# nguyenduchuyiu/marl-delivery

Measured on AMD Instinct MI355X. Metric: agent-steps/sec (whole node), map1 5-agent 4096 envs, 1/2/4/8 MI355X, higher is better.
Workload: dtype int32+fp64

## Files before the change

marl-delivery_amd/csrc/mdl_device.hpp:

```cpp
#pragma once
#include <hip/hip_runtime.h>
#include <stdint.h>

#if !defined(MDL_PROFILING_BUILD) && \
    (defined(MDL_EXP_NOWAIT) || defined(MDL_EXP_NOTUPLES) || defined(MDL_EXP_NOLDS) || defined(MDL_ABLATE) || \
     defined(MDL_STAMPS))
#error "MDL_EXP_NOWAIT / MDL_EXP_NOTUPLES / MDL_EXP_NOLDS / MDL_ABLATE / MDL_STAMPS need -DMDL_PROFILING_BUILD"
#endif
#ifndef MDL_ABLATE
#define MDL_ABLATE 0
#endif

namespace mdl {

constexpr int WAVE = 64;
constexpr int MT_N = 624;
constexpr int MT_M = 397;
constexpr int MAX_MAPS = 8;
constexpr int PKG_PAD = 256;

enum : int { ST_NONE = 0, ST_WAITING = 1, ST_IN_TRANSIT = 2, ST_DELIVERED = 3 };
enum : int { MV_S = 0, MV_L = 1, MV_R = 2, MV_U = 3, MV_D = 4, MV_OTHER = 5 };
enum : int { SH_PICK = 0, SH_ONTIME, SH_LATE, SH_CLOSER, SH_WPICK, SH_WDROP, SH_STUCK, SH_IDLE, SH_AWAY };

struct MapDesc {
    int H, W, nfree;
    int grid_off;
    int free_off;
    int rank_off;
    float inv_hw;
    int bits_off;
    int mvc_off;
};

struct __align__(16) EnvScalars {
    int32_t t;
    uint32_t ctr;
    double total;
};
enum : uint32_t { RT_MOVE = 1u, RT_ONTIME = 2u, RT_LATE = 4u };

enum : uint32_t { PS_STATUS = 3u, PS_PRESENT = 4u, PS_TRANSIT = 8u, PS_SURVIVOR = 16u, PS_FLAGS = 31u };
constexpr int PS_RANK_SHIFT = 5;

constexpr uint32_t ORD_EPISODE = 0x400u;

struct DevParams {
    int E, A, P, T;
    double move_cost, delivery_reward, delay_reward;
    double cost_sum[9];
    float shaping[9];
    int stale;
    int obsT, MO, MP, MR, MPs;
    int n_maps;
    int key32_dsh;
    MapDesc maps[MAX_MAPS];
    const uint8_t* grids;
    const uint8_t* movevalid;
    const uint8_t* movevalid_cell;
    const uint32_t* gridbits;
    const uint16_t* free_cells;
    const uint16_t* rank;
    const uint8_t* env_map;
    uint32_t* rob;
    uint64_t* pkg;
    uint16_t* pstate;
    EnvScalars* es;
    uint32_t* mt;
    int32_t* mt_pos;
    uint64_t* trk;
    double* ep_total;
    int32_t* ep_len;
    const double* obs_recip;
    int obs_plane_words;
    int obs_small;
    int key7_dsh;
    double cost_fold[65];
};

__host__ __device__ __forceinline__ uint32_t rob_pack(int cell, int carry, uint32_t valid_mask ) {
    return (uint32_t)cell | ((uint32_t)carry << 16) | ((valid_mask & 0x1eu) << 26);
}
__host__ __device__ __forceinline__ int rob_cell(uint32_t w) { return (int)(w & 0xffffu); }
__host__ __device__ __forceinline__ int rob_carry(uint32_t w) { return (int)((w >> 16) & 0x7ffu); }
__host__ __device__ __forceinline__ uint32_t rob_valid(uint32_t w) { return (w >> 26) & 0x1eu; }

__device__ __forceinline__ int lane_id() { return (int)(threadIdx.x & 63); }
__device__ __forceinline__ int wave_id() { return __builtin_amdgcn_readfirstlane((int)(threadIdx.x >> 6)); }

__device__ __forceinline__ int xcd_slot(int b, int nb) { return (b & 7) * (nb >> 3) + min(b & 7, nb & 7) + (b >> 3); }
__device__ __forceinline__ int xcd_block() {
    return xcd_slot((int)blockIdx.x, (int)gridDim.x);
}

__device__ __forceinline__ void wave_sync() {
    __builtin_amdgcn_fence(__ATOMIC_RELEASE, "wavefront");
    __builtin_amdgcn_wave_barrier();
    __builtin_amdgcn_fence(__ATOMIC_ACQUIRE, "wavefront");
}

__device__ __forceinline__ uint64_t ballot(bool p) { return __ballot(p); }

#define GLOBAL __attribute__((address_space(1)))
typedef unsigned int u32x4 __attribute__((ext_vector_type(4)));

template <class T>
__device__ __forceinline__ void pin(T& v) { asm volatile("" : "+s"(v)); }

__device__ __forceinline__ int rdl(int v, int j) { return __builtin_amdgcn_readlane(v, j); }
__device__ __forceinline__ float rdlf(float v, int j) {
    return __int_as_float(__builtin_amdgcn_readlane(__float_as_int(v), j));
}
__device__ __forceinline__ int uni(int v) { return __builtin_amdgcn_readfirstlane(v); }

__device__ __forceinline__ uint32_t lmask(bool b) {
    uint32_t x = b ? ~0u : 0u;
    asm("" : "+v"(x));
    return x;
}
__device__ __forceinline__ uint32_t vbit(uint64_t m, int lane) { return 0u - (uint32_t)((m >> lane) & 1ull); }
__device__ __forceinline__ float fmask(uint32_t m, float a) { return __uint_as_float(m & __float_as_uint(a)); }
__device__ __forceinline__ float fpick(uint32_t m, float a, float b) {
    return __uint_as_float((m & __float_as_uint(a)) | (~m & __float_as_uint(b)));
}
__device__ __forceinline__ int ipick(uint32_t m, int a, int b) { return (int)((m & (uint32_t)a) | (~m & (uint32_t)b)); }

__device__ __forceinline__ int popc64(uint64_t m) { return __popcll(m); }
__device__ __forceinline__ int ffs64(uint64_t m) { return __ffsll((long long)m) - 1; }
__device__ __forceinline__ uint64_t lanemask_lt() {
    int l = lane_id();
    return l == 0 ? 0ull : (~0ull >> (64 - l));
}

__device__ __forceinline__ uint32_t wave_min_u32(uint32_t v) {
    const int id = (int)0xffffffff;
    uint32_t t;
    t = (uint32_t)__builtin_amdgcn_update_dpp(id, (int)v, 0x111, 0xf, 0xf, false); v = t < v ? t : v;
    t = (uint32_t)__builtin_amdgcn_update_dpp(id, (int)v, 0x112, 0xf, 0xf, false); v = t < v ? t : v;
    t = (uint32_t)__builtin_amdgcn_update_dpp(id, (int)v, 0x114, 0xf, 0xf, false); v = t < v ? t : v;
    t = (uint32_t)__builtin_amdgcn_update_dpp(id, (int)v, 0x118, 0xf, 0xf, false); v = t < v ? t : v;
    t = (uint32_t)__builtin_amdgcn_update_dpp(id, (int)v, 0x142, 0xa, 0xf, false); v = t < v ? t : v;
    t = (uint32_t)__builtin_amdgcn_update_dpp(id, (int)v, 0x143, 0xc, 0xf, false); v = t < v ? t : v;
    return (uint32_t)__builtin_amdgcn_readlane((int)v, 63);
}

__device__ __forceinline__ void wave_min_u32x2(uint32_t u, uint32_t v, uint32_t& mu, uint32_t& mv) {
    const int id = (int)0xffffffff;
    uint32_t a, b;
#define MDL_MIN2(ctl, rm)                                                                  \
    a = (uint32_t)__builtin_amdgcn_update_dpp(id, (int)u, ctl, rm, 0xf, false);            \
    b = (uint32_t)__builtin_amdgcn_update_dpp(id, (int)v, ctl, rm, 0xf, false);            \
    u = a < u ? a : u;                                                                     \
    v = b < v ? b : v;
    MDL_MIN2(0x111, 0xf)
    MDL_MIN2(0x112, 0xf)
    MDL_MIN2(0x114, 0xf)
    MDL_MIN2(0x118, 0xf)
    MDL_MIN2(0x142, 0xa)
    MDL_MIN2(0x143, 0xc)
#undef MDL_MIN2
    mu = (uint32_t)__builtin_amdgcn_readlane((int)u, 63);
    mv = (uint32_t)__builtin_amdgcn_readlane((int)v, 63);
}

__device__ __forceinline__ int wave_min8_lane(int a) { return ((a >> 1) << 4) | ((a & 1) << 3); }
__device__ __forceinline__ uint32_t wave_min8_u32(const uint32_t (&k)[8]) {
    uint32_t m[4], n[2];
#pragma unroll
    for (int i = 0; i < 4; i++) {
        const auto r = __builtin_amdgcn_permlane32_swap(k[i], k[i + 4], false, false);
        m[i] = r[0] < r[1] ? r[0] : r[1];
    }
#pragma unroll
    for (int i = 0; i < 2; i++) {
        const auto r = __builtin_amdgcn_permlane16_swap(m[i], m[i + 2], false, false);
        n[i] = r[0] < r[1] ? r[0] : r[1];
    }
    const bool hi = (lane_id() & 8) != 0;
    const uint32_t keep = hi ? n[1] : n[0], send = hi ? n[0] : n[1];
    const int id = (int)0xffffffff;
    uint32_t t = (uint32_t)__builtin_amdgcn_update_dpp(id, (int)send, 0x128, 0xf, 0xf, false);
    uint32_t v = t < keep ? t : keep;
    t = (uint32_t)__builtin_amdgcn_update_dpp(id, (int)v, 0x141, 0xf, 0xf, false);
    v = t < v ? t : v;
    t = (uint32_t)__builtin_amdgcn_update_dpp(id, (int)v, 0x4E, 0xf, 0xf, false);
    v = t < v ? t : v;
    t = (uint32_t)__builtin_amdgcn_update_dpp(id, (int)v, 0xB1, 0xf, 0xf, false);
    return t < v ? t : v;
}

__device__ __forceinline__ float qdiv_r(int a, double y) { return (float)((double)a * y); }

__device__ __forceinline__ float qdiv(int a, int b) { return (float)a / (float)b; }

__device__ __forceinline__ int fdivi(int i, int d, float inv) {
    int q = (int)((float)i * inv);
    int r = i - q * d;
    if (r < 0) q -= 1;
    else if (r >= d) q += 1;
    return q;
}

__device__ __forceinline__ int cell_r(int pc) { return pc & 255; }
__device__ __forceinline__ int cell_c(int pc) { return (pc >> 8) & 255; }
__device__ __forceinline__ int manhattan(int a, int b) {
    return abs(cell_r(a) - cell_r(b)) + abs(cell_c(a) - cell_c(b));
}
__device__ __forceinline__ int manhattan_sad(int a, int b) {
    return (int)__builtin_amdgcn_sad_u8((uint32_t)a, (uint32_t)b, 0u);
}

__device__ __forceinline__ int pk_start(uint64_t v) { return (int)(v & 0xffff); }
__device__ __forceinline__ int pk_target(uint64_t v) { return (int)((v >> 16) & 0xffff); }
__device__ __forceinline__ int pk_st(uint64_t v) { return (int)((v >> 32) & 0xffff); }
__device__ __forceinline__ int pk_dl(uint64_t v) { return (int)(v >> 48); }
__device__ __forceinline__ uint64_t pk_make(int start, int target, int st, int dl) {
    return (uint64_t)(uint32_t)start | ((uint64_t)(uint32_t)target << 16) | ((uint64_t)(uint32_t)st << 32) |
           ((uint64_t)(uint32_t)dl << 48);
}

__device__ __forceinline__ void decode_action(int a, int fmt, int& mv, int& op) {
    if (fmt == 0) {
        const int q = a / 5;
        const int m = a - 5 * q;
        mv = (0x30214 >> (4 * m)) & 0xf;
        op = q >= 3 ? 0 : q;
    } else {
        mv = a & 7;
        op = (a >> 3) & 3;
        if (mv > MV_OTHER) mv = MV_OTHER;
    }
}

__device__ inline void mt_twist(uint32_t* key) {
    const int lane = lane_id();
    for (int base = 0; base < MT_N; base += WAVE) {
        const int i = base + lane;
        uint32_t v = 0;
        if (i < MT_N) {
            const uint32_t y = (key[i] & 0x80000000u) | (key[i + 1 == MT_N ? 0 : i + 1] & 0x7fffffffu);
            const int k = i + MT_M < MT_N ? i + MT_M : i + MT_M - MT_N;
            v = key[k] ^ (y >> 1) ^ ((y & 1u) ? 0x9908b0dfu : 0u);
        }
        wave_sync();
        if (i < MT_N) key[i] = v;
        wave_sync();
    }
}

struct MTState {
    uint32_t* key;
    int pos;
};

__device__ inline uint32_t mt_next32(MTState& s) {
    if (s.pos == MT_N) {
        mt_twist(s.key);
        s.pos = 0;
    }
    uint32_t y = s.key[s.pos];
    s.pos++;
    y ^= (y >> 11);
    y ^= (y << 7) & 0x9d2c5680u;
    y ^= (y << 15) & 0xefc60000u;
    y ^= (y >> 18);
    return (uint32_t)uni((int)y);
}

__device__ inline int randint(MTState& s, int lo, int hi) {
    const uint32_t rng = (uint32_t)(hi - 1 - lo);
    if (rng == 0) return lo;
    uint32_t mask = rng;
    mask |= mask >> 1; mask |= mask >> 2; mask |= mask >> 4; mask |= mask >> 8; mask |= mask >> 16;
    uint32_t v;
    do {
        v = mt_next32(s) & mask;
    } while (v > rng);
    return lo + (int)v;
}

struct ResetOut {
    int robot_cell;
};

__device__ inline int reset_env(MTState& mt, const DevParams& p, const MapDesc& md, uint64_t* pk, uint8_t* pst,
                                uint64_t* scratch, uint16_t* taken) {
    const int lane = lane_id();
    const int A = p.A, P = p.P;
    const uint16_t* fl = p.free_cells + md.free_off;
    const int F = md.nfree;
    int my_cell = 0;
    int ntk = 0;
    for (int i = 0; i < A; i++) {
        const int k = randint(mt, 0, F - i);
        int idx = k;
        for (int q = 0; q < ntk; q++) {
            const int tq = taken[q];
            if (tq <= idx) idx++;
            else break;
        }
        if (lane == 0) {
            int q = ntk;
            while (q > 0 && taken[q - 1] > idx) {
                taken[q] = taken[q - 1];
                q--;
            }
            taken[q] = (uint16_t)idx;
        }
        ntk++;
        wave_sync();
        if (lane == i) my_cell = fl[idx];
    }
    const int N = md.H;
    const int lim = A < 20 ? A : 20;
    for (int i = 0; i < P; i++) {
        const int s_idx = randint(mt, 0, F);
        int t_idx;
        do {
            t_idx = randint(mt, 0, F);
        } while (t_idx == s_idx);
        const int to_dl = 10 + randint(mt, N / 2, 3 * N);
        const int st = (i <= lim) ? 0 : randint(mt, 1, p.T);
        if (lane == 0) scratch[i] = pk_make(s_idx, t_idx, st, st + to_dl);
    }
    wave_sync();
    for (int j = lane; j < P; j += WAVE) {
        const uint64_t v = scratch[j];
        scratch[j] = pk_make(fl[pk_start(v)], fl[pk_target(v)], pk_st(v), pk_dl(v));
    }
    wave_sync();
    for (int j0 = 0; j0 < P; j0 += WAVE) {
        const int j = j0 + lane;
        uint64_t v = 0;
        int sj = 0, rank = 0;
        if (j < P) {
            v = scratch[j];
            sj = pk_st(v);
        }
        for (int i = 0; i < P; i++) {
            const int si = pk_st(scratch[i]);
            rank += (si < sj) || (si == sj && i < j);
        }
        if (j < P) {
            pk[rank] = v;
        }
    }
    wave_sync();
    for (int j = lane; j < P; j += WAVE) pst[j] = pk_st(pk[j]) == 0 ? ST_WAITING : ST_NONE;
    wave_sync();
    return my_cell;
}

struct TrkFresh {
    static constexpr bool kIdIndexed = true;
    const uint64_t* pk;
    const uint8_t* ps;
    int n;
    __device__ int count() const { return n; }
    __device__ bool present(int j) const { const int s = ps[j] & PS_STATUS; return s == ST_WAITING || s == ST_IN_TRANSIT; }
    __device__ bool in_transit(int j) const { return (ps[j] & PS_STATUS) == ST_IN_TRANSIT; }
    __device__ uint64_t data(int j) const { return pk[j]; }
    __device__ int id(int j) const { return j + 1; }
    __device__ uint32_t order(int j) const { return (uint32_t)j; }
    __device__ int slot_of(int id) const { return (id >= 1 && id <= n && present(id - 1)) ? id - 1 : -1; }
};

struct TrkStale {
    static constexpr bool kIdIndexed = true;
    const uint8_t* ps;
    const uint64_t* td;
    const uint32_t* tq;
    int n;
    __device__ int count() const { return n; }
    __device__ bool present(int j) const { return (ps[j] & PS_PRESENT) != 0; }
    __device__ bool in_transit(int j) const { return (ps[j] & PS_TRANSIT) != 0; }
    __device__ uint64_t data(int j) const { return td[j]; }
    __device__ int id(int j) const { return j + 1; }
    __device__ uint32_t order(int j) const { return tq[j]; }
    __device__ int slot_of(int id) const { return (id >= 1 && id <= n && present(id - 1)) ? id - 1 : -1; }
};

struct TrkView {
    static constexpr bool kIdIndexed = false;
    const int32_t* ids;
    const uint8_t* flag;
    const uint64_t* pk;
    int n;
    __device__ int count() const { return n; }
    __device__ bool present(int j) const { return flag[j] & 1; }
    __device__ bool in_transit(int j) const { return (flag[j] & 2) != 0; }
    __device__ uint64_t data(int j) const { return pk[j]; }
    __device__ int id(int j) const { return ids[j]; }
    __device__ uint32_t order(int j) const { return (uint32_t)j; }
    __device__ int slot_of(int id) const {
        for (int j = 0; j < n; j++)
            if (ids[j] == id) return j;
        return -1;
    }
};

template <class Trk>
__device__ inline float shaped_agent(const Trk& trk, const float* C, bool active, int prev_cell, int prev_carry,
                                     int cur_cell, int cur_carry, int mv, int op, int t_prev, int t_cur) {
    float s = 0.0f;
    const int pslot = (active && prev_carry != 0) ? trk.slot_of(prev_carry) : -1;
    if (prev_carry == 0 && cur_carry != 0) {
        s = s + C[SH_PICK];
    } else if (prev_carry != 0 && cur_carry == 0) {
        if (pslot >= 0) {
            const uint64_t d = trk.data(pslot);
            if (cur_cell == pk_target(d)) s = s + ((t_cur <= pk_dl(d)) ? C[SH_ONTIME] : C[SH_LATE]);
        }
    }
    const bool moved = prev_cell != cur_cell;
    const bool need_can = active && op == 1 && prev_carry == 0 && cur_carry == 0;
    const bool need_near = active && moved && !(prev_carry != 0 && pslot >= 0);
    const bool need_idle = active && !moved && mv == MV_S && prev_carry == 0;
    bool can = false, idle = false;
    int best_d = 0x7fffffff;
    uint32_t best_o = 0xffffffffu;
    int best_cell = -1;
    if (__ballot(need_can || need_near || need_idle)) {
        const int n = trk.count();
        for (int j = 0; j < n; j++) {
            if (!trk.present(j) || trk.in_transit(j)) continue;
            const uint64_t d = trk.data(j);
            if (pk_st(d) > t_prev) continue;
            const int sc = pk_start(d);
            can |= sc == cur_cell;
            const int md = manhattan(prev_cell, sc);
            idle |= md <= 3;
            const uint32_t o = trk.order(j);
            if (md < best_d || (md == best_d && o < best_o)) {
                best_d = md;
                best_o = o;
                best_cell = sc;
            }
        }
    }
    if (op == 1) {
        if (prev_carry != 0) s = s + C[SH_WPICK];
        else if (cur_carry == 0 && !can) s = s + C[SH_WPICK];
    } else if (op == 2) {
        if (prev_carry == 0) s = s + C[SH_WDROP];
        else if (cur_carry != 0 && pslot >= 0 && cur_cell != pk_target(trk.data(pslot))) s = s + C[SH_WDROP];
    }
    if (mv != MV_S && !moved) s = s + C[SH_STUCK];
    int target = -1;
    if (prev_carry != 0 && pslot >= 0) target = pk_target(trk.data(pslot));
    else target = best_cell;
    if (target >= 0 && moved) {
        const int db = manhattan(prev_cell, target), da = manhattan(cur_cell, target);
        if (da < db) s = s + C[SH_CLOSER];
        else if (da > db) s = s + C[SH_AWAY];
    }
    if (!moved && mv == MV_S && prev_carry == 0 && idle) s = s + C[SH_IDLE];
    return active ? s : 0.0f;
}

template <int AU>
__device__ inline float np_sum_lanes8(float v, int n) {
    static_assert(AU >= 1 && AU <= 8, "np_sum_lanes8: 1 <= AU <= 8");
    float x[8];
#pragma unroll
    for (int i = 0; i < 8; i++) x[i] = i < AU ? rdlf(v, i) : 0.0f;
    float res;
    if (AU == 8 && n == 8) {
        res = ((x[0] + x[1]) + (x[2] + x[3])) + ((x[4] + x[5]) + (x[6] + x[7]));
    } else {
        res = 0.0f;
#pragma unroll
        for (int i = 0; i < (AU < 7 ? AU : 7); i++) res = res + x[i];
    }
    return 0.0f + res;
}

__device__ inline float np_sum_lanes(float v, int n) {
    float res;
    if (n < 8) {
        res = 0.0f;
        for (int i = 0; i < n; i++) res = res + rdlf(v, i);
    } else {
        float r0 = rdlf(v, 0), r1 = rdlf(v, 1), r2 = rdlf(v, 2), r3 = rdlf(v, 3);
        float r4 = rdlf(v, 4), r5 = rdlf(v, 5), r6 = rdlf(v, 6), r7 = rdlf(v, 7);
        int i;
        for (i = 8; i < n - (n % 8); i += 8) {
            r0 = r0 + rdlf(v, i + 0); r1 = r1 + rdlf(v, i + 1); r2 = r2 + rdlf(v, i + 2); r3 = r3 + rdlf(v, i + 3);
            r4 = r4 + rdlf(v, i + 4); r5 = r5 + rdlf(v, i + 5); r6 = r6 + rdlf(v, i + 6); r7 = r7 + rdlf(v, i + 7);
        }
        res = ((r0 + r1) + (r2 + r3)) + ((r4 + r5) + (r6 + r7));
        for (; i < n; i++) res = res + rdlf(v, i);
    }
    return 0.0f + res;
}

template <int AU>
__device__ inline float np_sum_lanes_dpp(float v) {
    static_assert(AU >= 1 && AU <= 7, "np_sum_lanes_dpp: 1 <= AU <= 7");
    float t = v;
#pragma unroll
    for (int i = 1; i < AU; i++) {
        const float prev = __int_as_float(__builtin_amdgcn_update_dpp(0, __float_as_int(t), 0x111, 0xf, 0xf, true));
        t = v + prev;
    }
    return rdlf(t, AU - 1);
}

template <int CTL>
__device__ __forceinline__ float dppf(float x) {
    return __int_as_float(__builtin_amdgcn_update_dpp(0, __float_as_int(x), CTL, 0xf, 0xf, true));
}
__device__ inline float np_sum16_dpp(float v) {
    const float r = v + dppf<0x128>(v);
    const float s = r + dppf<0xB1>(r);
    const float c = s + dppf<0x4E>(s);
    const float d = c + dppf<0x124>(c);
    return 0.0f + rdlf(d, 0);
}

template <int AU>
__device__ inline float np_sum_step(float v, int n) {
    if constexpr (AU > 0 && AU <= 7) return np_sum_lanes_dpp<AU>(v);
    else if constexpr (AU == 16) return np_sum16_dpp(v);
    else if constexpr (AU == 8) return np_sum_lanes8<AU>(v, n);
    else return np_sum_lanes(v, n);
}

}
```

marl-delivery_amd/csrc/mdl_kernels.hip:

```cpp
#include <cstring>
#include <type_traits>

#include "mdl_kernels.hpp"
#include "mdl_features.hpp"
#include "mdl_obs_small.hpp"
#include "mdl_altfeat.hpp"


namespace mdl {

#ifdef MDL_STAMPS
__device__ uint64_t g_stamps[65536 * 16];
#define STAMP(k)                                      \
    do {                                              \
        __builtin_amdgcn_sched_barrier(0);            \
        stamp_[k] = __builtin_amdgcn_s_memtime();     \
        __builtin_amdgcn_sched_barrier(0);            \
    } while (0)
#else
#define STAMP(k) \
    do {         \
    } while (0)
#endif

__host__ __device__ inline int stage_floats(int A, int na, int MO, int MPc, int MR, int MPsc) {
    const int dc = actor_compact_dim(A, MO, MPc);
    const int a = actor_group(na, dc) * dc, cr = critic_compact_dim(A, MR, MPsc);
    return a > cr ? a : cr;
}

struct ResetLds {
    uint64_t* pk;
    uint64_t* scratch;
    uint32_t* mt;
    uint16_t* taken;
    uint8_t* pst;
};

__host__ __device__ constexpr size_t reset_lds_bytes(int P) {
    return align16(8 * (size_t)P) * 2 + align16(4 * MT_N) + align16(2 * 64) + align16((size_t)P);
}

__device__ inline ResetLds reset_carve(unsigned char* b, int P) {
    ResetLds L;
    size_t o = 0;
    L.pk = (uint64_t*)(b + o); o += align16(8 * (size_t)P);
    L.scratch = (uint64_t*)(b + o); o += align16(8 * (size_t)P);
    L.mt = (uint32_t*)(b + o); o += align16(4 * MT_N);
    L.taken = (uint16_t*)(b + o); o += align16(2 * 64);
    L.pst = b + o;
    return L;
}

__device__ inline void load_mt(const DevParams& p, int e, uint32_t* key) {
    const uint32_t* g = p.mt + (size_t)e * MT_N;
    for (int i = lane_id(); i < MT_N; i += WAVE) key[i] = g[i];
    wave_sync();
}

__device__ inline void store_mt(const DevParams& p, int e, const uint32_t* key, int pos) {
    uint32_t* g = p.mt + (size_t)e * MT_N;
    for (int i = lane_id(); i < MT_N; i += WAVE) g[i] = key[i];
    if (lane_id() == 0) p.mt_pos[e] = pos;
}

__device__ inline int do_reset(const DevParams& p, int e, const MapDesc& md, ResetLds& L, bool seeded_in_lds) {
    if (!seeded_in_lds) load_mt(p, e, L.mt);
    MTState ms{L.mt, seeded_in_lds ? MT_N : p.mt_pos[e]};
    const int cell = reset_env(ms, p, md, L.pk, L.pst, L.scratch, L.taken);
    store_mt(p, e, L.mt, ms.pos);
    return cell;
}

template <int NCH, int AU = 0>
__device__ inline void tracker_update_regs(uint32_t (&ps)[NCH], uint64_t (&td)[NCH], bool (&dirty)[NCH],
                                           const uint64_t (&pk)[NCH], int P, int A, int carry, int t) {
    const int lane = lane_id();
#pragma unroll
    for (int c = 0; c < NCH; c++) {
        const int j = c * WAVE + lane;
        const bool ins = (j < P) & (pk_st(pk[c]) == t) & !(ps[c] & PS_PRESENT);
        ps[c] = ins ? ((ps[c] & PS_STATUS) | PS_PRESENT) : ps[c];
        td[c] = ins ? pk[c] : td[c];
        dirty[c] = dirty[c] || ins;
    }
#pragma unroll
    for (int c = 0; c < NCH; c++) {
        const int id = c * WAVE + lane + 1;
        bool carried = false;
        if constexpr (AU > 0) {
            uint32_t ci[AU], mn = 0xffffffffu;
#pragma unroll
            for (int i = 0; i < AU; i++) ci[i] = (uint32_t)rdl(carry, i);
            __builtin_amdgcn_sched_barrier(0);
#pragma unroll
            for (int i = 0; i < AU; i++) mn = min(mn, ci[i] ^ (uint32_t)id);
            carried = mn == 0u;
        } else {
            for (int i = 0; i < A; i++) carried |= rdl(carry, i) == id;
        }
        const uint32_t upd = carried ? (ps[c] | PS_TRANSIT) : (ps[c] & PS_TRANSIT) ? (ps[c] & PS_STATUS) : ps[c];
        ps[c] = (ps[c] & PS_PRESENT) ? upd : ps[c];
    }
}

template <int NCH>
__device__ inline void tracker_update_bits(uint32_t (&ps)[NCH], uint64_t (&td)[NCH], bool (&dirty)[NCH],
                                           const uint64_t (&pk)[NCH], int P, int t, uint32_t carried_bits) {
    const int lane = lane_id();
#pragma unroll
    for (int c = 0; c < NCH; c++) {
        const int j = c * WAVE + lane;
        const bool ins = (j < P) & (pk_st(pk[c]) == t) & !(ps[c] & PS_PRESENT);
        ps[c] = ins ? ((ps[c] & PS_STATUS) | PS_PRESENT) : ps[c];
        td[c] = ins ? pk[c] : td[c];
        dirty[c] = dirty[c] || ins;
        const bool carried = (carried_bits >> c) & 1u;
        const uint32_t upd = carried ? (ps[c] | PS_TRANSIT) : (ps[c] & PS_TRANSIT) ? (ps[c] & PS_STATUS) : ps[c];
        ps[c] = (ps[c] & PS_PRESENT) ? upd : ps[c];
    }
}

template <int NCH>
__device__ inline void survivors_at_reset(uint32_t (&ps)[NCH], uint32_t (&tq)[NCH], int P) {
    const int lane = lane_id();
    uint32_t rk[NCH];
#pragma unroll
    for (int c = 0; c < NCH; c++) rk[c] = 0;
#pragma unroll
    for (int c2 = 0; c2 < NCH; c2++) {
        uint64_t m = ballot(c2 * WAVE + lane < P && (ps[c2] & PS_PRESENT));
        while (m) {
            const uint32_t ki = (uint32_t)rdl((int)tq[c2], ffs64(m));
            m &= m - 1;
#pragma unroll
            for (int c = 0; c < NCH; c++) rk[c] += ki < tq[c] ? 1u : 0u;
        }
    }
#pragma unroll
    for (int c = 0; c < NCH; c++) {
        if (c * WAVE + lane < P && (ps[c] & PS_PRESENT)) {
            tq[c] = rk[c];
            ps[c] = (ps[c] & PS_FLAGS) | PS_SURVIVOR | (rk[c] << PS_RANK_SHIFT);
        } else {
            ps[c] &= PS_STATUS;
        }
    }
}

__global__ __launch_bounds__(256) void k_seed(DevParams p, const uint32_t* __restrict__ seeds, int wpb,
                                              int lds_stride) {
    extern __shared__ __align__(16) unsigned char smem[];
    const int wave = wave_id();
    const int lane = lane_id();
    const int e = blockIdx.x * wpb + wave;
    if (wave >= wpb || e >= p.E) return;
    ResetLds L = reset_carve(smem + (size_t)wave * lds_stride, p.P);
    const MapDesc md = p.maps[p.env_map ? p.env_map[e] : 0];
    if (lane == 0) {
        uint32_t s = seeds[e];
        for (int i = 0; i < MT_N; i++) {
            L.mt[i] = s;
            s = 1812433253u * (s ^ (s >> 30)) + (uint32_t)(i + 1);
        }
    }
    wave_sync();
    const int cell = do_reset(p, e, md, L, true);
    if (lane < p.A)
        p.rob[(size_t)e * p.A + lane] = rob_pack(cell, 0, p.movevalid[md.grid_off + cell_r(cell) * md.W + cell_c(cell)]);
    for (int j = lane; j < p.P; j += WAVE) {
        const size_t g = (size_t)e * p.P + j;
        p.pkg[g] = L.pk[j];
        p.pstate[g] = L.pst[j];
    }
    if (lane == 0) {
        EnvScalars s;
        s.t = 0;
        s.ctr = 0;
        s.total = 0.0;
        p.es[e] = s;
        p.ep_total[e] = 0.0;
        p.ep_len[e] = 0;
    }
}

template <int NCH>
__global__ __launch_bounds__(256) void k_reset(DevParams p, const int* __restrict__ env_ids, int n, int wpb,
                                               int lds_stride) {
    extern __shared__ __align__(16) unsigned char smem[];
    const int wave = wave_id();
    const int lane = lane_id();
    const int w = xcd_block() * wpb + wave;
    if (wave >= wpb || w >= n) return;
    const int e = env_ids ? env_ids[w] : w;
    if ((unsigned)e >= (unsigned)p.E) return;
    const int A = p.A, P = p.P;
    ResetLds L = reset_carve(smem + (size_t)wave * lds_stride, P);
    const MapDesc md = p.maps[p.env_map ? p.env_map[e] : 0];
    uint32_t ps[NCH], tq[NCH];
#pragma unroll
    for (int c = 0; c < NCH; c++) {
        const int j = c * WAVE + lane;
        ps[c] = j < P ? p.pstate[(size_t)e * P + j] : 0u;
        tq[c] = (p.stale && (ps[c] & PS_SURVIVOR)) ? ps[c] >> PS_RANK_SHIFT : ORD_EPISODE + (uint32_t)j;
    }
    const int cell = do_reset(p, e, md, L, false);
    uint64_t pk[NCH], td[NCH];
    bool dirty[NCH];
    if (p.stale) survivors_at_reset<NCH>(ps, tq, P);
#pragma unroll
    for (int c = 0; c < NCH; c++) {
        const int j = c * WAVE + lane;
        pk[c] = j < P ? L.pk[j] : 0;
        ps[c] = (j < P ? L.pst[j] : 0u) | (p.stale ? (ps[c] & ~PS_STATUS) : 0u);
        td[c] = pk[c];
        dirty[c] = false;
    }
    if (p.stale) tracker_update_regs<NCH>(ps, td, dirty, pk, P, A, 0, 0);
    if (lane < A)
        p.rob[(size_t)e * A + lane] = rob_pack(cell, 0, p.movevalid[md.grid_off + cell_r(cell) * md.W + cell_c(cell)]);
#pragma unroll
    for (int c = 0; c < NCH; c++) {
        const int j = c * WAVE + lane;
        if (j < P) {
            const size_t g = (size_t)e * P + j;
            p.pkg[g] = pk[c];
            p.pstate[g] = (uint16_t)ps[c];
            if (dirty[c]) p.trk[g] = td[c];
        }
    }
    if (lane == 0) {
        EnvScalars s;
        s.t = 0;
        s.ctr = 0;
        s.total = 0.0;
        p.es[e] = s;
    }
}

__global__ __launch_bounds__(256) void k_tracker_clear(DevParams p, const int* __restrict__ env_ids, int n) {
    const int wave = wave_id();
    const int w = blockIdx.x * 4 + wave;
    if (w >= n) return;
    const int e = env_ids ? env_ids[w] : w;
    if ((unsigned)e >= (unsigned)p.E) return;
    for (int j = lane_id(); j < p.P; j += WAVE) {
        const size_t g = (size_t)e * p.P + j;
        p.pstate[g] &= (uint16_t)PS_STATUS;
    }
    if (lane_id() == 0) p.es[e].ctr = 0;
}

#define MDL_STEP_LB 256
template <int NCH, bool FUSED>
constexpr int step_wpe() { return (NCH <= 2 && !FUSED) ? 8 : 1; }
#define MDL_STEP_ATTR(NCH, FUSED) __attribute__((amdgpu_waves_per_eu(step_wpe<NCH, FUSED>())))
struct StepArgs {
    DevParams p;
    const uint8_t* actions;
    const int* env_ids;
    double* r_out;
    float* sh_out;
    uint8_t* done_out;
    int fmt, n, auto_reset, wpb, lds_stride, K;
};
typedef __attribute__((address_space(4))) const StepArgs* KargPtr;
static_assert(sizeof(StepArgs) + 256 <= 4096, "the step's kernel arguments stay inside the 4 KiB kernarg segment");

struct StepKarg {
    const uint32_t* rob;
    const uint64_t* pkg;
    const uint16_t* pst;
    const u32x4* es;
    const uint64_t* trk;
    const uint8_t* act;
    uint32_t ap, nw;
    StepArgs args;
};
constexpr uint32_t NW_IDS = 1u << 29, NW_MAP = 1u << 30;
constexpr uint32_t NW_SMALLMAP = 1u << 31;
constexpr int AP_NB_SHIFT = 18;
inline uint32_t pack_ap(int A, int P, int nblocks) {
    const uint32_t nb = nblocks < (1 << (32 - AP_NB_SHIFT)) ? (uint32_t)nblocks : 0u;
    return (uint32_t)A | ((uint32_t)P << 7) | (nb << AP_NB_SHIFT);
}

struct ObsArgs {
    float* amap;
    float* avec;
    float* cmap;
    float* cvec;
};

struct EpiArgs {
    uint8_t* active;
    uint8_t* filled;
};
typedef __attribute__((address_space(4))) const EpiArgs* EpiKargPtr;
constexpr size_t EPI_KARG_OFF = sizeof(StepArgs) + sizeof(ObsArgs);
static_assert(sizeof(StepArgs) % 8 == 0 && sizeof(ObsArgs) % 8 == 0, "EpiArgs starts where ObsArgs ends");

__device__ __forceinline__ void publish_tail(const Publish& pb) {
    __atomic_thread_fence(__ATOMIC_RELEASE);
    if (!pb.ctr) {
        if (lane_id() == 0) __hip_atomic_store(pb.seq, pb.value, __ATOMIC_RELAXED, __HIP_MEMORY_SCOPE_SYSTEM);
        return;
    }
    if (lane_id() == 0) {
        const unsigned waves = pb.expect ? pb.expect : gridDim.x * (blockDim.x / WAVE);
        if (atomicAdd(pb.ctr, 1u) - pb.base == waves - 1u) {
            __atomic_thread_fence(__ATOMIC_ACQ_REL);
            __hip_atomic_store(pb.seq, pb.value, __ATOMIC_RELEASE, __HIP_MEMORY_SCOPE_SYSTEM);
        }
    }
}

constexpr int MAIL_INLINE_CODES = 256;
struct MailArgs {
    MailRows m;
    Publish pb;
    uint8_t codes[MAIL_INLINE_CODES];
};

#include "mdl_step_common.hpp"

__host__ __device__ constexpr uint64_t move_lt_lanes(int k) {
    uint64_t m = 0;
    for (int l = 0; l < 64; l++)
        if (((l >> 4) << 2) + k < (l & 15)) m |= 1ull << l;
    return m;
}

template <bool STALE, int NCH, bool FUSED, int AU, bool OBS, bool MAIL = false, bool EPI = false>
__device__ __forceinline__ void step_body(const uint32_t* __restrict__ rob_pre, const uint64_t* __restrict__ pkg_pre,
                                          const uint16_t* __restrict__ pst_pre, const u32x4* __restrict__ es_pre,
                                          const uint64_t* __restrict__ trk_pre, const uint8_t* __restrict__ act_pre,
                                          uint32_t ap, uint32_t nw, const StepArgs& args, const ObsArgs& oa,
                                          const MailArgs* ma = nullptr) {
    static_assert(!OBS || (NCH == 1 && !FUSED && AU > 0 && AU <= 8), "fused observations: P <= 64, A <= 8");
    static_assert(!EPI || (OBS && !MAIL), "the episode form is the fused step + observation launch's");
    extern __shared__ __align__(16) unsigned char smem[];
    const DevParams& p = args.p;
#ifdef MDL_STAMPS
    uint64_t stamp_[16];
#endif
    STAMP(0);
    const int A = (int)(ap & 0x7fu), P = (int)((ap >> 7) & 0x7ffu);
    const int n_ = (int)(nw & 0xffffffu), wpb_ = (int)((nw >> 24) & 31u);
    GLOBAL const uint32_t* robp = (GLOBAL const uint32_t*)rob_pre;
    GLOBAL const uint64_t* pkgp = (GLOBAL const uint64_t*)pkg_pre;
    GLOBAL const uint16_t* pstp = (GLOBAL const uint16_t*)pst_pre;
    GLOBAL const u32x4* esp = (GLOBAL const u32x4*)es_pre;
    GLOBAL const uint64_t* trkp = (GLOBAL const uint64_t*)trk_pre;
    GLOBAL const uint8_t* actp = (GLOBAL const uint8_t*)act_pre;
    STAMP(1);

    const int wave = wave_id();
    const int lane = lane_id();
    const int nbp = (int)(ap >> AP_NB_SHIFT);
    const int w = (nbp ? xcd_slot((int)blockIdx.x, nbp) : (int)blockIdx.x) * wpb_ + wave;
    if (wave >= wpb_ || w >= n_) return;
    int e = w;
    if (nw & NW_IDS) {
        e = uni(((GLOBAL const int*)args.env_ids)[w]);
        if ((unsigned)e >= (unsigned)args.p.E) return;
    }
    if constexpr (EPI) {
        KargPtr ka = (KargPtr)((__attribute__((address_space(4))) const char*)
                                   __builtin_amdgcn_kernarg_segment_ptr() + offsetof(StepKarg, args));
        asm volatile("" : "+s"(ka));
        EpiKargPtr ke = (EpiKargPtr)((__attribute__((address_space(4))) const char*)ka + EPI_KARG_OFF);
        if (!uni((int)((GLOBAL const uint8_t*)ke->active)[w])) {
            if (lane == 0) {
// ... 1542 lines not shown
```

Before: 4.948 billion.

## Wave-parallel Mersenne Twister rejection sampling and ballot-based reset sampling

Replaces the serial per-draw MT19937 tempering and rejection loop with a wave-wide stream: each lane tempers one key word and ballots mask-accept flags for the common draw ranges, so a draw becomes a find-first-set over a bitmask. Agent cell selection with taken-index skipping uses ballot and popcount instead of an LDS sorted list, and the package rank sort compares packed 32-bit keys through lane reads instead of rereading LDS. The MT key is written back to global memory only when a twist happened. This aims to cut serial latency and LDS traffic in environment reset. It adds complexity around keeping the exact RNG sequence and position, including the edge case where a start-time range is empty.

```diff
diff --git a/marl-delivery_amd/csrc/mdl_device.hpp b/marl-delivery_amd/csrc/mdl_device.hpp
--- a/marl-delivery_amd/csrc/mdl_device.hpp
+++ b/marl-delivery_amd/csrc/mdl_device.hpp
@@ -234,6 +234,7 @@
 
 __device__ inline void mt_twist(uint32_t* key) {
     const int lane = lane_id();
+#pragma unroll 1
     for (int base = 0; base < MT_N; base += WAVE) {
         const int i = base + lane;
         uint32_t v = 0;
@@ -248,79 +249,118 @@
     }
 }
 
-struct MTState {
+enum : int { DRAW_CELL = 0, DRAW_SPAN = 1, DRAW_START = 2, DRAW_KINDS = 3 };
+struct MTStream {
     uint32_t* key;
-    int pos;
-};
-
-__device__ inline uint32_t mt_next32(MTState& s) {
-    if (s.pos == MT_N) {
-        mt_twist(s.key);
-        s.pos = 0;
-    }
-    uint32_t y = s.key[s.pos];
-    s.pos++;
+    int base;
+    int twists;
+    uint32_t w;
+    uint64_t live;
+    uint32_t rng[DRAW_KINDS];
+    uint64_t acc[DRAW_KINDS];
+};
+
+__device__ __forceinline__ uint32_t draw_mask(uint32_t rng) { return ~0u >> __builtin_clz(rng); }
+__device__ __forceinline__ uint64_t mt_window_lanes(int base) { return ~0ull >> (WAVE - min(WAVE, MT_N - base)); }
+
+__device__ inline void mt_fill(MTStream& s) {
+    uint32_t y = s.key[min(s.base + lane_id(), MT_N - 1)];
     y ^= (y >> 11);
     y ^= (y << 7) & 0x9d2c5680u;
     y ^= (y << 15) & 0xefc60000u;
     y ^= (y >> 18);
-    return (uint32_t)uni((int)y);
-}
-
-__device__ inline int randint(MTState& s, int lo, int hi) {
-    const uint32_t rng = (uint32_t)(hi - 1 - lo);
-    if (rng == 0) return lo;
-    uint32_t mask = rng;
-    mask |= mask >> 1; mask |= mask >> 2; mask |= mask >> 4; mask |= mask >> 8; mask |= mask >> 16;
-    uint32_t v;
-    do {
-        v = mt_next32(s) & mask;
-    } while (v > rng);
-    return lo + (int)v;
-}
-
-struct ResetOut {
-    int robot_cell;
-};
-
-__device__ inline int reset_env(MTState& mt, const DevParams& p, const MapDesc& md, uint64_t* pk, uint8_t* pst,
-                                uint64_t* scratch, uint16_t* taken) {
+    s.w = y;
+    const uint64_t valid = mt_window_lanes(s.base);
+#pragma unroll
+    for (int k = 0; k < DRAW_KINDS; k++) s.acc[k] = ballot((y & draw_mask(s.rng[k])) <= s.rng[k]) & valid;
+}
+
+__device__ inline MTStream mt_open(uint32_t* key, int pos, uint32_t rng_cell, uint32_t rng_span, uint32_t rng_start) {
+    MTStream s;
+    s.key = key;
+    s.base = pos & ~(WAVE - 1);
+    s.twists = 0;
+    s.rng[DRAW_CELL] = rng_cell;
+    s.rng[DRAW_SPAN] = rng_span;
+    s.rng[DRAW_START] = rng_start;
+    mt_fill(s);
+    s.live = ~0ull << (pos & (WAVE - 1));
+    return s;
+}
+
+__device__ __forceinline__ int mt_pos(const MTStream& s) {
+    const uint64_t m = s.live & mt_window_lanes(s.base);
+    return m ? s.base + ffs64(m) : min(s.base + WAVE, MT_N);
+}
+
+__device__ inline void mt_refill(MTStream& s) {
+    s.base += WAVE;
+    if (s.base >= MT_N) {
+        mt_twist(s.key);
+        s.base = 0;
+        s.twists++;
+    }
+    mt_fill(s);
+    s.live = ~0ull;
+}
+
+__device__ __forceinline__ int mt_take(MTStream& s, uint64_t m, uint32_t rng) {
+    const int l = ffs64(m);
+    s.live = ~1ull << l;
+    return (int)((uint32_t)rdl((int)s.w, l) & draw_mask(rng));
+}
+template <int K>
+__device__ inline int mt_draw(MTStream& s) {
+    for (;;) {
+        const uint64_t m = s.acc[K] & s.live;
+        if (m) return mt_take(s, m, s.rng[K]);
+        mt_refill(s);
+    }
+}
+__device__ inline int mt_draw_rng(MTStream& s, uint32_t rng) {
+    for (;;) {
+        const uint64_t m = ballot((s.w & draw_mask(rng)) <= rng) & mt_window_lanes(s.base) & s.live;
+        if (m) return mt_take(s, m, rng);
+        mt_refill(s);
+    }
+}
+
+__device__ inline MTStream reset_stream(uint32_t* key, int pos, const DevParams& p, const MapDesc& md) {
+    const int N = md.H;
+    return mt_open(key, pos, (uint32_t)(md.nfree - 1), (uint32_t)(3 * N - 1 - N / 2), (uint32_t)max(p.T - 2, 1));
+}
+
+__device__ inline int reset_env(MTStream& mt, const DevParams& p, const MapDesc& md, uint64_t* pk, uint8_t* pst,
+                                uint64_t* scratch) {
     const int lane = lane_id();
     const int A = p.A, P = p.P;
     const uint16_t* fl = p.free_cells + md.free_off;
     const int F = md.nfree;
-    int my_cell = 0;
-    int ntk = 0;
+    __builtin_assume(A >= 1 && P >= 1 && F >= 2);
+    int tk = 0x7fffffff;
     for (int i = 0; i < A; i++) {
-        const int k = randint(mt, 0, F - i);
+        const int k = F - 1 - i > 0 ? mt_draw_rng(mt, (uint32_t)(F - 1 - i)) : 0;
         int idx = k;
-        for (int q = 0; q < ntk; q++) {
-            const int tq = taken[q];
-            if (tq <= idx) idx++;
-            else break;
-        }
-        if (lane == 0) {
-            int q = ntk;
-            while (q > 0 && taken[q - 1] > idx) {
-                taken[q] = taken[q - 1];
-                q--;
-            }
-            taken[q] = (uint16_t)idx;
-        }
-        ntk++;
-        wave_sync();
-        if (lane == i) my_cell = fl[idx];
-    }
+        for (;;) {
+            const int nx = k + popc64(ballot(tk <= idx));
+            if (nx == idx) break;
+            idx = nx;
+        }
+        tk = lane == i ? idx : tk;
+    }
+    const int my_cell = lane < A ? fl[tk] : 0;
     const int N = md.H;
     const int lim = A < 20 ? A : 20;
+    const int lim_draw = p.T > 2 ? lim : P;
     for (int i = 0; i < P; i++) {
-        const int s_idx = randint(mt, 0, F);
+        const int s_idx = mt_draw<DRAW_CELL>(mt);
         int t_idx;
         do {
-            t_idx = randint(mt, 0, F);
+            t_idx = mt_draw<DRAW_CELL>(mt);
         } while (t_idx == s_idx);
-        const int to_dl = 10 + randint(mt, N / 2, 3 * N);
-        const int st = (i <= lim) ? 0 : randint(mt, 1, p.T);
+        const int to_dl = 10 + N / 2 + mt_draw<DRAW_SPAN>(mt);
+        int st = i <= lim ? 0 : 1;
+        if (i > lim_draw) st += mt_draw<DRAW_START>(mt);
         if (lane == 0) scratch[i] = pk_make(s_idx, t_idx, st, st + to_dl);
     }
     wave_sync();
@@ -329,24 +369,22 @@
         scratch[j] = pk_make(fl[pk_start(v)], fl[pk_target(v)], pk_st(v), pk_dl(v));
     }
     wave_sync();
+    const uint32_t* st_word = (const uint32_t*)scratch;
     for (int j0 = 0; j0 < P; j0 += WAVE) {
         const int j = j0 + lane;
-        uint64_t v = 0;
-        int sj = 0, rank = 0;
+        const uint32_t kj = j < P ? (st_word[2 * j + 1] << 16) | (uint32_t)j : 0u;
+        int rank = 0;
+        for (int i0 = 0; i0 < P; i0 += WAVE) {
+            const int ii = i0 + lane;
+            const uint32_t ki = ii < P ? (st_word[2 * ii + 1] << 16) | (uint32_t)ii : ~0u;
+            const int ni = min(WAVE, P - i0);
+            for (int l = 0; l < ni; l++) rank += (uint32_t)rdl((int)ki, l) < kj;
+        }
         if (j < P) {
-            v = scratch[j];
-            sj = pk_st(v);
-        }
-        for (int i = 0; i < P; i++) {
-            const int si = pk_st(scratch[i]);
-            rank += (si < sj) || (si == sj && i < j);
-        }
-        if (j < P) {
-            pk[rank] = v;
-        }
-    }
-    wave_sync();
-    for (int j = lane; j < P; j += WAVE) pst[j] = pk_st(pk[j]) == 0 ? ST_WAITING : ST_NONE;
+            pk[rank] = scratch[j];
+            pst[rank] = (kj >> 16) == 0 ? ST_WAITING : ST_NONE;
+        }
+    }
     wave_sync();
     return my_cell;
 }
diff --git a/marl-delivery_amd/csrc/mdl_kernels.hip b/marl-delivery_amd/csrc/mdl_kernels.hip
--- a/marl-delivery_amd/csrc/mdl_kernels.hip
+++ b/marl-delivery_amd/csrc/mdl_kernels.hip
@@ -33,12 +33,11 @@
     uint64_t* pk;
     uint64_t* scratch;
     uint32_t* mt;
-    uint16_t* taken;
     uint8_t* pst;
 };
 
 __host__ __device__ constexpr size_t reset_lds_bytes(int P) {
-    return align16(8 * (size_t)P) * 2 + align16(4 * MT_N) + align16(2 * 64) + align16((size_t)P);
+    return align16(8 * (size_t)P) * 2 + align16(4 * MT_N) + align16((size_t)P);
 }
 
 __device__ inline ResetLds reset_carve(unsigned char* b, int P) {
@@ -47,7 +46,6 @@
     L.pk = (uint64_t*)(b + o); o += align16(8 * (size_t)P);
     L.scratch = (uint64_t*)(b + o); o += align16(8 * (size_t)P);
     L.mt = (uint32_t*)(b + o); o += align16(4 * MT_N);
-    L.taken = (uint16_t*)(b + o); o += align16(2 * 64);
     L.pst = b + o;
     return L;
 }
@@ -58,17 +56,19 @@
     wave_sync();
 }
 
-__device__ inline void store_mt(const DevParams& p, int e, const uint32_t* key, int pos) {
-    uint32_t* g = p.mt + (size_t)e * MT_N;
-    for (int i = lane_id(); i < MT_N; i += WAVE) g[i] = key[i];
+__device__ inline void store_mt(const DevParams& p, int e, const uint32_t* key, int pos, bool keys) {
+    if (keys) {
+        uint32_t* g = p.mt + (size_t)e * MT_N;
+        for (int i = lane_id(); i < MT_N; i += WAVE) g[i] = key[i];
+    }
     if (lane_id() == 0) p.mt_pos[e] = pos;
 }
 
 __device__ inline int do_reset(const DevParams& p, int e, const MapDesc& md, ResetLds& L, bool seeded_in_lds) {
     if (!seeded_in_lds) load_mt(p, e, L.mt);
-    MTState ms{L.mt, seeded_in_lds ? MT_N : p.mt_pos[e]};
-    const int cell = reset_env(ms, p, md, L.pk, L.pst, L.scratch, L.taken);
-    store_mt(p, e, L.mt, ms.pos);
+    MTStream ms = reset_stream(L.mt, seeded_in_lds ? MT_N : uni(p.mt_pos[e]), p, md);
+    const int cell = reset_env(ms, p, md, L.pk, L.pst, L.scratch);
+    store_mt(p, e, L.mt, mt_pos(ms), ms.twists > 0 || seeded_in_lds);
     return cell;
 }
 
```

Result: no change. 4.949 billion, median of 3 (+0.0%).
